# cgmb/euler

Measured on AMD Instinct MI355X. Metric: cells*steps/sec of sim_step() (frames incl. the PCG pressure projection) + pressure-solve HBM GB/s vs roofline, higher is better.
Workload: dtype f64

## Files before the change

euler_amd/__init__.py:

```python
import ctypes as C
import os

import numpy as np

_HERE = os.path.dirname(os.path.abspath(__file__))
LIB_PATH = os.path.join(_HERE, "lib", "libeuler_hip.so")

DOT_AUTO, DOT_SEQUENTIAL, DOT_TREE = 0, 1, 2
PRECOND_IC0, PRECOND_JACOBI, PRECOND_IC0_TILE, PRECOND_IC0_TILE2, PRECOND_IC0_TILE_MG = 0, 1, 2, 3, 4
(OPT_P_STEPS, OPT_TILE_STORE_AS, OPT_TILE_REVERSE, OPT_RESIDENT_CAP, OPT_GRID4_MIN_CELLS, OPT_SLAB_FUSION, OPT_RCCL_SMALL, OPT_RCCL_NO_EXCHANGE, OPT_MARKERS_ROWMAJOR,
 OPT_SA_RUN, OPT_NO_INTERIOR, OPT_BUILD_GATHER, OPT_RESIDENT_FORCE_TIMEOUT, OPT_MG_SPLIT_LEVEL, OPT_MG_SPLIT_ACTIVE, OPT_MARKERS_TWO_PASS, OPT_BUILD_TWO_PASS,
 OPT_VELOCITY_TWO_PASS, OPT_NO_TILE_MAP, OPT_PROFILE_STRIDE, OPT_TILE_STORE_Z, OPT_ADVECT_RK2, OPT_ADVECT_MACCORMACK) = range(1, 24)
SWEEP_AUTO, SWEEP_BAND, SWEEP_SIMPLE = 0, 1, 2
PCG_F64, PCG_F32 = 0, 1
RESIDENT_AUTO, RESIDENT_OFF = 0, 1
IMAGE_COVERAGE, IMAGE_DYE, IMAGE_SPEED = 0, 1, 2
EDIT_SOLID, EDIT_CLEAR, EDIT_SINK, EDIT_SOURCE, EDIT_FILL, EDIT_DRAIN = range(6)
OVERVIEW_DTYPE = np.dtype({"names": ["cells", "solid", "sink", "water", "marks", "max_speed2", "dye"],
                           "formats": [np.uint32, np.uint32, np.uint32, np.uint32, np.uint32, np.float32, (np.uint64, 3)],
                           "offsets": [0, 4, 8, 12, 16, 20, 24], "itemsize": 48})
DIAG_CROWDED = 8
DIAG_DTYPE = np.dtype({"names": ["cells", "fluid", "markers", "crowded", "mass_x", "mass_y", "div_l1", "ke_hi", "ke_lo", "count_max", "nonfinite", "max_div", "max_speed2"],
                       "formats": [np.uint64] * 9 + [np.uint32, np.uint32, np.float32, np.float32],
                       "offsets": [0, 8, 16, 24, 32, 40, 48, 56, 64, 72, 76, 80, 84], "itemsize": 88})
FLOW_PRESSURE = 1
PAINT_VORTICITY, PAINT_PRESSURE, PAINT_SPEED = 0, 1, 2
FLOW_DTYPE = np.dtype({"names": ["cells", "water", "nodes", "nonfinite", "u_pos", "u_neg", "v_pos", "v_neg", "w_pos", "w_neg", "p_sum", "max_speed2", "max_abs_w", "max_p", "reserved"],
# ... 891 lines not shown
```

euler_amd/csrc/driver.hip:

```cpp
#include "euler_dev.h"
#include "k_mg.h"

#include <math.h>
#include <stdarg.h>
#include <stdlib.h>
#include <string.h>

#include <vector>

int eu_launch_build_system(euler_sim* S, float dt);
int eu_launch_velocity_update(euler_sim* S, float dt, int finish);
int eu_pressure_current(euler_sim* S);
int eu_unskew(euler_sim* S, const void* skew, void* rowmajor, int elem_bytes);
int eu_unskew_fluid(euler_sim* S, const double* skew, double* rowmajor);
double* eu_current_search_direction(euler_sim* S);
int eu_launch_tile_table(euler_sim* S);
int eu_skew(euler_sim* S, const void* rowmajor, void* skew, int elem_bytes);
int eu_set_source_count(euler_sim* S, size_t nsrc);

static thread_local char g_err[512] = "";

void eu_set_error(const char* fmt, ...) {
  va_list ap;
  va_start(ap, fmt);
// ... 108 lines not shown

bool eu_resident_eligible(const euler_sim* S) {
  if (S->res_disabled || S->cfg.resident == EULER_RESIDENT_OFF) return false;
  if (S->cfg.precond != EULER_PRECOND_IC0_TILE || S->tile_w != 16 || S->cfg.sweep_mode == EULER_SWEEP_SIMPLE || S->cfg.dot_mode != EULER_DOT_TREE) return false;
  if (S->has_comm || S->slab_on || S->p2p_on) return false;
  const int cap = eu_resident_capacity(const_cast<euler_sim*>(S), S->cfg.pcg_precision == EULER_PCG_F32);
  if (S->cfg.pcg_precision == EULER_PCG_F32) return cap > 0 && S->geom.nbands * (S->geom.T / 16) <= 4 * cap;
  return cap > 0;
}
extern "C" int euler_resident_info(euler_sim* S, uint64_t out[3]) {
  if (!S || !out) return EULER_EINVAL;
  out[0] = eu_resident_eligible(S) ? 1 : 0; out[1] = S->res_solves; out[2] = S->res_fallbacks;
  return EULER_OK;
}

extern "C" int euler_set_option(euler_sim* S, int32_t key, int64_t value) {
  if (!S || key <= 0 || key >= EULER_OPT__COUNT) { eu_set_error("euler_set_option: unknown key %d", (int)key); return EULER_EINVAL; }
  bool ok = true;
  const char* when = nullptr;
  switch (key) {
    case EULER_OPT_P_STEPS: ok = value == 2 || value == 4 || value == 8; break;
    case EULER_OPT_SA_RUN: ok = value == 8 || value == 16 || value == 32;
      if (ok && value != 8 && (S->has_comm || eu_is_two_level(S))) when = "on a handle without a communicator, in the parity or the plain tile-local mode (the others run runs of 8)";
      break;
    case EULER_OPT_RCCL_SMALL: ok = value >= 0 && value <= 2; if (S->rccl) when = "before euler_set_comm_rccl"; break;
    case EULER_OPT_RCCL_NO_EXCHANGE: ok = value == 0 || value == 1; if (S->rccl) when = "before euler_set_comm_rccl"; break;
    case EULER_OPT_SLAB_FUSION: ok = value == 0 || value == 1; if (S->p2p_on) when = "before euler_p2p_connect"; break;
    case EULER_OPT_RESIDENT_CAP: case EULER_OPT_GRID4_MIN_CELLS: case EULER_OPT_RESIDENT_FORCE_TIMEOUT: ok = value >= 0; break;
    case EULER_OPT_MG_SPLIT_LEVEL: ok = value >= -1 && value < 12; break;
    case EULER_OPT_PROFILE_STRIDE: ok = value >= 1 && value <= 1024; break;
    case EULER_OPT_MG_SPLIT_ACTIVE: ok = false; break;
    case EULER_OPT_ADVECT_RK2: ok = value == 0 || value == 1;
// ... 15 lines not shown
      eu_set_error("euler_set_option: EULER_OPT_ADVECT_MACCORMACK needs %zu bytes of scratch", 2 * bytes);
      return EULER_ENOMEM;
    }
    S->mc_u = a; S->mc_v = b;
  }
  if (key == EULER_OPT_P_STEPS || key == EULER_OPT_SA_RUN) {
    int rcp = eu_pressure_current(S);
    if (rcp) return rcp;
  }
  S->opt[key] = value;
  if (key == EULER_OPT_P_STEPS || key == EULER_OPT_SA_RUN) S->s_ring_n = 0;
  if (key == EULER_OPT_MG_SPLIT_LEVEL) { eu_mg_split_release(S); S->opt[EULER_OPT_MG_SPLIT_ACTIVE] = 0; }
  return EULER_OK;
}
extern "C" int euler_get_option(euler_sim* S, int32_t key, int64_t* value) {
  if (!S || !value || key <= 0 || key >= EULER_OPT__COUNT) { eu_set_error("euler_get_option: unknown key %d", (int)key); return EULER_EINVAL; }
  *value = S->opt[key];
  return EULER_OK;
}

static const char* eu_precond_combination(const euler_sim* S, int precond, int tile_w, int has_comm, int slab_on, int p2p_on) {
  const bool coarse = precond == EULER_PRECOND_IC0_TILE2 || precond == EULER_PRECOND_IC0_TILE_MG;
  if (!coarse) return nullptr;
  if (tile_w != 16 || S->cfg.sweep_mode == EULER_SWEEP_SIMPLE) return "the coarse-correction preconditioners run on tiles of 16 records with the band schedule";
  if (precond == EULER_PRECOND_IC0_TILE2 && (has_comm || slab_on)) return "EULER_PRECOND_IC0_TILE2 runs on one GPU (row slabs: EULER_PRECOND_IC0_TILE_MG)";
  if (precond == EULER_PRECOND_IC0_TILE_MG && has_comm && (!slab_on || p2p_on)) return "EULER_PRECOND_IC0_TILE_MG with several ranks: row-slab handles without mailboxes only";
  return nullptr;
}

extern "C" int euler_set_precond(euler_sim* S, int32_t precond, int32_t tile_records) {
  if (!S || precond < EULER_PRECOND_IC0 || precond > EULER_PRECOND_IC0_TILE_MG) { eu_set_error("euler_set_precond: bad argument"); return EULER_EINVAL; }
// ... 884 lines not shown
```

euler_amd/csrc/k_grid.hip:

```cpp
#include "k_pcg.h"
#include "k_transport.h"

#include <stdlib.h>

__device__ __forceinline__ void dt_from_maxima(MarkerState* ms, float frame_time_left, unsigned int mu_bits, unsigned int mv_bits) {
  const float mu = __uint_as_float(mu_bits), mv = __uint_as_float(mv_bits);
  const float max_distance = 0.75f * EU_H;
  const float max_velocity = sqrtf(mu + mv);
  ms->dt = fminf(max_distance / max_velocity, frame_time_left);
  ms->max_u2_bits = 0u;
  ms->max_v2_bits = 0u;
}
template <bool FUSE_DT>
__global__ __launch_bounds__(256) void k_maxsq(const float* __restrict__ u, const float* __restrict__ v,
                                               int X, int Y, MarkerState* ms, int y0, int y1, float frame_time_left) {
  float mu = 0.f, mv = 0.f;
  const bool vec = (X & 3) == 0;
  for (int yq = y0 + 4 * (int)blockIdx.x; yq < y1; yq += 4 * (int)gridDim.x) {
    if (vec) {
      for (int x = 4 * (int)threadIdx.x; x < X; x += 4 * 256) {
        float4 a[4], b[4];
#pragma unroll
        for (int r = 0; r < 4; ++r) {
          const int y = yq + r < y1 ? yq + r : y1 - 1;
// ... 662 lines not shown
    const bool f1 = count[i + X] != 0;
    float o = 0.f;
    if (solid[i] | solid[i + X]) o = 0.f;
    else if (f0 | f1) {
      double p1 = p[skew_index(g, x, y + 1)];
      if (f1 && p1 < 0.0) p1 = 0.0;
      o = vin[i] + (neg_inv * (float)(p1 - p0)) * dt;
    }
    vout[i] = o;
  }
}

struct VuRing { const double* s[8]; int n, steps, use; };
#define VU_W 48
#define VU_ILP 4
__global__ __launch_bounds__(256) void k_velocity_update_para(const float* __restrict__ uin, const float* __restrict__ vin, float* __restrict__ uout, float* __restrict__ vout,
                                                              const double* __restrict__ p, const uint8_t* __restrict__ mask, const uint8_t* __restrict__ count,
                                                              const uint8_t* __restrict__ solid, SkewGeom g, float dt, const PcgScalars* sc, VuRing ring, MarkerState* ms,
                                                              int band_lo, int do_max, int skip_zero,
                                                              const uint8_t* __restrict__ tmap, int tnx) {
  __shared__ double sp[65][VU_W + 1];
  __shared__ float s_mu[4], s_mv[4];
  const int units = g.T / VU_W;
  const size_t blk = eu_xcd_block();
  const int band = band_lo + (int)(blk / units), t0 = (int)(blk % units) * VU_W;
  const int X = g.X, Y = g.Y, tid = threadIdx.x;
  if (skip_zero && tmap && eu_tiles_idle_cur(tmap, tnx, band, t0 > 63 ? (t0 - 63) >> 6 : 0, (t0 + VU_W - 1) >> 6, true)) return;
  int cnt = 0, from = 0;
  if (ring.use && sc->nonzero && sc->iters > 0) {
    const int n_it = sc->iters;
    from = n_it - 1 >= ring.steps ? (n_it - 1) / ring.steps * ring.steps : 0;
    cnt = n_it - from;
  }
  double al[8];
  const double* sq[8];
#pragma unroll
  for (int j = 0; j < 8; ++j) { const int it = from + (j < cnt ? j : 0); al[j] = sc->alpha_hist[it & 7]; sq[j] = ring.s[it % ring.n]; }
  const size_t ebase = ((size_t)band * g.TS + (size_t)t0) * 64;
  static_assert((64 * VU_W) % (256 * VU_ILP) == 0, "whole rounds of VU_ILP elements per thread");
  for (int c0 = tid; c0 < 64 * VU_W; c0 += 256 * VU_ILP) {
    uint8_t m[VU_ILP];
    double pv[VU_ILP];
    bool any = false;
#pragma unroll
    for (int u = 0; u < VU_ILP; ++u) { m[u] = mask[ebase + (size_t)(c0 + 256 * u)]; any = any || (m[u] & CM_FLUID); }
    if (__any(any)) {
#pragma unroll
      for (int u = 0; u < VU_ILP; ++u) pv[u] = p[ebase + (size_t)(c0 + 256 * u)];
#pragma unroll
      for (int j = 0; j < 8; ++j)
        if (j < cnt) {
          double sv[VU_ILP];
#pragma unroll
          for (int u = 0; u < VU_ILP; ++u) sv[u] = sq[j][ebase + (size_t)(c0 + 256 * u)];
// ... 156 lines not shown
  if (!mode) return EULER_OK;
  eu_vd_pressure_made_current(&S->vd);
  if (mode == 1) { int rc = eu_launch_finish_p(S); if (rc) return rc; }
  LAUNCH(S, KC_VELOCITY_UPDATE, k_clamp_p, dim3(eu_blocks(S->e_cnt, 256 * 4, 4096)), dim3(256), S->p, S->cellmask, S->e_lo, S->e_cnt);
  return EULER_OK;
}
int eu_launch_velocity_update(euler_sim* S, float dt, int finish) {
  const bool one_pass = (!S->has_comm || S->slab_on) && S->opt[EULER_OPT_VELOCITY_TWO_PASS] == 0 && (!S->slab_on || !finish);
  if (one_pass) {
    VuRing ring;
    for (int k = 0; k < 8; ++k) ring.s[k] = S->s_ring[k < S->s_ring_n ? k : 0];
    ring.n = S->s_ring_n > 0 ? S->s_ring_n : 1; ring.steps = ring.n; ring.use = finish && S->s_ring_n > 0;
    if (!ring.use) for (int k = 0; k < 8; ++k) ring.s[k] = S->p;
    const int do_max = S->slab_on ? 0 : 1;
    if (eu_vd_update_clears_maxima(&S->vd, do_max)) HIPCHK(hipMemsetAsync(&S->ms->max_u2_bits, 0, 2 * sizeof(unsigned int), S->stream));
    LAUNCH(S, KC_VELOCITY_UPDATE, k_velocity_update_para, dim3((unsigned)((size_t)(S->band_hi - S->band_lo) * (S->geom.T / VU_W))), dim3(256), S->utmp, S->vtmp, S->u, S->v, S->p, S->cellmask,
           S->count, S->solid, S->geom, dt, S->sc, ring, S->ms, S->band_lo, do_max, eu_vd_update_skips_zeros(&S->vd, S->slab_on),
           eu_tile_map_on(S) ? (const uint8_t*)S->tmap : (const uint8_t*)nullptr, S->tmap_nx);
    eu_vd_velocity_updated(&S->vd, 1, ring.use, do_max);
    return EULER_OK;
  }
  if (finish) { int rc = eu_launch_finish_p(S); if (rc) return rc; }
  dim3 grid((S->X + 63) / 64, (S->row_hi - S->row_lo + 3) / 4);
  LAUNCH(S, KC_VELOCITY_UPDATE, k_velocity_update, grid, dim3(256), S->utmp, S->vtmp, S->u, S->v, S->p, S->count,
         S->solid, S->geom, dt, S->row_lo, S->row_hi);
  eu_vd_velocity_updated(&S->vd, 0, 0, 0);
  return EULER_OK;
}

template <typename T>
__global__ __launch_bounds__(256) void k_unskew(const T* __restrict__ skew, T* __restrict__ rowmajor, SkewGeom g, int y0, int y1) {
// ... 33 lines not shown
```

euler_amd/csrc/k_pcg.h:

```cpp
#pragma once

#include "euler_dev.h"
#include "k_mg.h"

#define COMM_CALL(expr) do { if ((expr) != 0) { eu_set_error("communicator callback failed: %s", #expr); return EULER_ECOMM; } } while (0)
#define LOC(ptr) ((ptr) + S->e_lo)
enum { SW_FACTOR = 0, SW_FORWARD = 1, SW_BACKWARD = 2 };

int eu_launch_build_system(euler_sim* S, float dt);
int eu_launch_velocity_update(euler_sim* S, float dt, int finish);
int eu_launch_band_ranges(euler_sim* S);
int eu_launch_sweep(euler_sim* S, int op, int cls, int force, int fin_qq = -1);
int eu_launch_factor_tile(euler_sim* S, int force);
int eu_launch_precond_tile(euler_sim* S, int rupd, int sweeps, int fin_dot, int force, double alpha, bool r_only = false, int zform = -1);
int eu_launch_search_apply(euler_sim* S, int it);
int eu_launch_finish_p(euler_sim* S);
int eu_launch_dot(euler_sim* S, const double* a, const double* b, int fin_op, int force);
int eu_comm_exchange(euler_sim* S, double* send_lo, double* send_hi, double* recv_lo, double* recv_hi, int count, double* small, int nsmall);
int eu_comm_finish(euler_sim* S, int fin_op, int is_max, int force);
int eu_comm_halo_two(euler_sim* S, double* a, double* b);
bool tile_recompute(const euler_sim* S);
int p_steps(const euler_sim* S);

enum { FIN_SIGMA_INIT = 0, FIN_ALPHA, FIN_RNORM, FIN_BETA, FIN_STORE_ONLY, FIN_TO_COMM };
#define FIN_VIA_P2P 0x100

static inline bool tile_fused(const euler_sim* S) { return eu_is_tile(S) && S->cfg.sweep_mode != EULER_SWEEP_SIMPLE; }
static inline bool ghost_mode(const euler_sim* S) { return S->has_comm && !S->p2p_on && tile_fused(S); }
enum { XR_ZSEND_LO = 0, XR_ZSEND_HI, XR_ZRECV_LO, XR_ZRECV_HI, XR_GS_LO0, XR_GS_LO1, XR_GS_HI0, XR_GS_HI1 };
// ... 189 lines not shown
  const unsigned int* list;
  const double* table;
  PcgScalars* sc;
  int force;
  double alpha_arg;
  double* pair_slot;
  double *zsend_lo, *zsend_hi;
  int edge_lo, edge_hi;
  int reverse;
  double* cpart;
  int cshift;
  int cmode, cnx, cny;
  const double *gs_lo, *gs_hi;
  int zform;
  double *zhalo, *zrows;
};

__device__ __forceinline__ double factor_step(double aa, double own, double nbv) {
  const double cl = -1.0 * own, cb = -1.0 * nbv;
  double e = aa - cl * cl - cb * cb;
  if (e < 0.25 * aa) e = (aa != 0.0) ? aa : 1.0;
  return 1.0 / sqrt(e);
}

template <int CTRL>
__device__ __forceinline__ double dpp_move(double v) {
  const int lo = __builtin_amdgcn_update_dpp(0, __double2loint(v), CTRL, 0xf, 0xf, true);
  const int hi = __builtin_amdgcn_update_dpp(0, __double2hiint(v), CTRL, 0xf, 0xf, true);
  return __hiloint2double(hi, lo);
}
// ... 8 lines not shown
```

euler_amd/csrc/k_pcg.hip:

```cpp
#include "k_pcg.h"

#include <cmath>
#include <vector>

template <bool IS_MAX>
__global__ __launch_bounds__(RED_THREADS) void k_reduce_final(const double* __restrict__ partial, int n, PcgScalars* sc,
                                                              int op, int force) {
  if (!force && pcg_idle(sc)) return;
  double v = 0.0;
  for (int i = threadIdx.x; i < n; i += RED_THREADS) {
    const double w = partial[i];
    if (IS_MAX) v = w > v ? w : v; else v += w;
  }
  v = IS_MAX ? block_max(v) : block_sum(v);
  if (threadIdx.x == 0) pcg_scalar_step(sc, op, v);
}

template <bool EDGES>
__global__ __launch_bounds__(RED_THREADS) void k_dot_partial(const double* __restrict__ a, const double* __restrict__ b,
                                                             const uint8_t* __restrict__ mask, size_t S,
                                                             double* __restrict__ partial, PcgScalars* sc, int force,
                                                             unsigned int* counter, int fin_op, int TS, int nb_local, int edges) {
  if (!force && pcg_idle(sc)) return;
  const size_t chunk = (((S + gridDim.x - 1) / gridDim.x) + 1) & ~(size_t)1;
// ... 49 lines not shown
      for (int grp = 0; grp < SEQ_TILE / 64; ++grp) {
        if (any[buf][grp] == 0ull) continue;
        const double* pp = &prod[buf][grp * 64];
        double v[64];
#pragma unroll
        for (int k = 0; k < 64; ++k) v[k] = pp[k];
#pragma unroll
        for (int k = 0; k < 64; ++k) total += v[k];
      }
    }
    __syncthreads();
  }
  if (threadIdx.x == 0) pcg_scalar_step(sc, op, total);
}

__global__ __launch_bounds__(RED_THREADS) void k_apply_a(const double* __restrict__ s, double* __restrict__ z,
                                                         const uint8_t* __restrict__ mask, SkewGeom g,
                                                         double* __restrict__ partial, PcgScalars* sc, int force,
                                                         unsigned int* counter, int fin_op) {
  if (!force && pcg_idle(sc)) return;
  const size_t S = g.S;
  const size_t chunk = (((S + gridDim.x - 1) / gridDim.x) + 127) & ~(size_t)127;
  const size_t lo = (size_t)blockIdx.x * chunk, hi = lo + chunk < S ? lo + chunk : S;
  double t = 0.0;
  for (size_t i = lo + 2 * (size_t)threadIdx.x; i < hi; i += 2 * RED_THREADS) {
    const unsigned int mm = *reinterpret_cast<const unsigned short*>(mask + i);
    const unsigned int m0 = mm & 0xff, m1 = mm >> 8;
    if (!((m0 | m1) & CM_FLUID)) continue;
    const sw_d2 c = *reinterpret_cast<const sw_d2*>(s + i);
    const int l = (int)((i & 127) >> 1);
// ... 28 lines not shown
        v = v - s[up];
      } else {
        v = v - 0.0;
      }
      v = v - ((m1 & CM_LEFT) ? c.x : 0.0);
      if (m1 & CM_DOWN) {
        size_t dn = i - 2;
        if (l == 0) { int band, tt, ll; skew_decode(g, i + 1, band, tt, ll); dn = skew_index(g, tt, 64 * band - 1); }
        v = v - s[dn];
      } else {
        v = v - 0.0;
      }
      o.y = v;
      t += v * c.y;
    }
    if ((m0 & m1) & CM_FLUID) *reinterpret_cast<sw_d2*>(z + i) = o;
    else if (m0 & CM_FLUID) z[i] = o.x;
    else z[i + 1] = o.y;
  }
  t = block_sum(t);
  if (fin_op >= 0) block_finish<false>(t, partial, counter, sc, fin_op);
}

__global__ __launch_bounds__(RED_THREADS) void k_update_pr(double* __restrict__ p, double* __restrict__ r,
                                                           const double* __restrict__ s, const double* __restrict__ z,
                                                           const uint8_t* __restrict__ mask, size_t S,
                                                           double* __restrict__ partial, PcgScalars* sc, int force,
                                                           double alpha_arg, unsigned int* counter, int fin_op) {
  if (!force && pcg_idle(sc)) return;
  const double alpha = force ? alpha_arg : sc->alpha;
// ... 224 lines not shown

static inline bool dot_rides_in_sweep(const euler_sim* S) { return S->cfg.precond == EULER_PRECOND_IC0 && S->cfg.sweep_mode != EULER_SWEEP_SIMPLE && !S->has_comm && S->cfg.dot_mode != EULER_DOT_SEQUENTIAL; }
static int launch_precondition(euler_sim* S, int force, int fin_dot = -1) {
  if (S->cfg.precond == EULER_PRECOND_JACOBI) {
    LAUNCH(S, KC_JACOBI, k_jacobi, dim3(eu_blocks(S->e_cnt, 256 * 4, 4096)), dim3(256), LOC(S->r), LOC(S->z), LOC(S->cellmask),
           S->e_cnt, S->sc, force);
    return fin_dot >= 0 ? eu_launch_dot(S, S->z, S->r, fin_dot, force) : EULER_OK;
  }
  const bool ride = fin_dot >= 0 && dot_rides_in_sweep(S);
  int rc = eu_launch_sweep(S, SW_FORWARD, KC_FORWARD_SOLVE, force, ride ? fin_dot : -1);
  if (rc) return rc;
  if ((rc = eu_launch_sweep(S, SW_BACKWARD, KC_BACKWARD_SOLVE, force))) return rc;
  return fin_dot >= 0 && !ride ? eu_launch_dot(S, S->z, S->r, fin_dot, force) : EULER_OK;
}

static int launch_apply_a_and_alpha(euler_sim* S, int force) {
  const bool seq = S->cfg.dot_mode == EULER_DOT_SEQUENTIAL && !S->has_comm;
  if (S->has_comm && ghost_mode(S) && !force) {
    const int X = S->X, nbk = (X + 255) / 256;
    const bool coarse = eu_is_two_level(S);
    if (S->band_lo > 0) {
      HIPCHK(hipMemcpyAsync(xrow(S, XR_GS_LO0), xrow(S, XR_ZRECV_LO), (size_t)X * 8, hipMemcpyDeviceToDevice, S->stream));
      if (coarse) { int rc = eu_launch_coarse_add_row(S, xrow(S, XR_GS_LO0), 64 * S->band_lo - 1); if (rc) return rc; }
      hipLaunchKernelGGL(k_unpack_row, dim3(nbk), dim3(256), 0, S->stream, S->s, xrow(S, XR_GS_LO0), S->geom, S->band_lo - 1, 63);
    }
    if (S->band_hi < S->geom.nbands) {
      HIPCHK(hipMemcpyAsync(xrow(S, XR_GS_HI0), xrow(S, XR_ZRECV_HI), (size_t)X * 8, hipMemcpyDeviceToDevice, S->stream));
      if (coarse) { int rc = eu_launch_coarse_add_row(S, xrow(S, XR_GS_HI0), 64 * S->band_hi); if (rc) return rc; }
      hipLaunchKernelGGL(k_unpack_row, dim3(nbk), dim3(256), 0, S->stream, S->s, xrow(S, XR_GS_HI0), S->geom, S->band_hi, 0);
    }
    S->gs_cur = 0;
  } else if (S->has_comm) { int rc = comm_halo_s(S); if (rc) return rc; }
  SkewGeom gl = S->geom;
  gl.S = S->e_cnt;
  double* out = tile_fused(S) ? S->q : S->z;
  LAUNCH(S, KC_APPLY_A, k_apply_a, dim3(loc_red_blocks(S)), dim3(RED_THREADS), LOC(S->s), LOC(out), LOC(S->cellmask), gl,
         S->partial, S->sc, force, S->red_counter, seq ? -1 : fin_or_comm(S, FIN_ALPHA));
  if (seq)
    LAUNCH(S, KC_DOT, k_dot_sequential, dim3(1), dim3(256), out, S->s, S->cellmask, S->geom, S->sc, (int)FIN_ALPHA, force);
  return S->has_comm ? eu_comm_finish(S, FIN_ALPHA, 0, force) : EULER_OK;
}

int p_steps(const euler_sim* S) {
  if (S->p2p_on || sa_run(S) != 8) return 2;
  return (int)S->opt[EULER_OPT_P_STEPS];
}
static int ring_begin(euler_sim* S) {
  const int n = p_steps(S);
  if (!S->s_base[0]) { S->s_base[0] = S->s; S->s_base[1] = S->s2; }
  if (n > 2) { S->s = S->s_base[0]; S->s2 = S->s_base[1]; }
  else if (S->s != S->s_base[0] && S->s != S->s_base[1]) { S->s = S->s_base[0]; S->s2 = S->s_base[1]; }
// ... 93 lines not shown
    }
  }
  return EULER_OK;
}

static int project_first_direction(euler_sim* S, Solve& v) {
  int rc;
  const bool tile = tile_fused(S), two_level = tile && eu_is_two_level(S);
  if (two_level && S->has_comm && !(eu_is_mg(S) && ghost_mode(S) && S->slab_on)) {
    eu_set_error("coarse-correction preconditioners with several ranks: EULER_PRECOND_IC0_TILE_MG on row slabs without mailboxes only");
    return EULER_EINVAL;
  }
  if (two_level && (rc = eu_launch_coarse_setup(S))) return rc;
  if (two_level && (rc = eu_launch_coarse_consistent(S))) return rc;
  v.zr = tile && tile_z_begin(S);
  if (tile) {
    if ((rc = eu_launch_factor_tile(S, 0))) return rc;
    if ((rc = eu_launch_precond_tile(S, 0, 1, FIN_SIGMA_INIT, 0, 0.0))) return rc;
  } else {
  if (S->cfg.precond != EULER_PRECOND_JACOBI && (rc = eu_launch_sweep(S, SW_FACTOR, KC_PRECON_FACTOR, 0))) return rc;
  if ((rc = launch_precondition(S, 0, FIN_SIGMA_INIT))) return rc;
  }
  if ((rc = ring_begin(S))) return rc;
  if (first_direction_folded(S)) {
    const PcgScalars& ps = v.prev;
    if (ps.nonzero && !(std::isfinite(ps.alpha) && std::isfinite(ps.beta) && std::isfinite(ps.rnorm) && std::isfinite(ps.sigma) && std::isfinite(ps.zs)))
      for (int k = 0; k < S->s_ring_n; ++k) HIPCHK(hipMemsetAsync(S->s_ring[k] + S->skew_off, 0, S->Sw * sizeof(double), S->stream));
  }
  else if (two_level) { if ((rc = eu_launch_coarse_search_init(S))) return rc; }
  else
  LAUNCH(S, KC_UPDATE_SEARCH, k_update_search<true>, dim3(eu_blocks(S->e_cnt, 256 * 4, 4096)), dim3(256), LOC(S->s), LOC(S->z),
         LOC(S->cellmask), S->e_cnt, S->sc, 0, 0.0);
  if (S->has_comm && eu_p2p_has_neighbour_arrays(S)) {
    const int y0 = S->band_lo > 0 ? 64 * S->band_lo : -1, y1 = S->band_hi < S->geom.nbands ? 64 * S->band_hi - 1 : -1;
    LAUNCH(S, KC_UPDATE_SEARCH, k_publish_edge_rows, dim3((S->X + 255) / 256, 2), dim3(256), S->s, S->geom, y0, y1, S->sc);
  }
  if (S->s_ring_n == 2) HIPCHK(hipMemsetAsync(LOC(S->s2), 0, S->e_cnt * sizeof(double), S->stream));
  S->s_stale = 1;
  return EULER_OK;
}

static int project_iterate(euler_sim* S, Solve& v) {
  int rc;
  HIPCHK(hipMemcpyAsync(S->sc_host, S->sc, sizeof(PcgScalars), hipMemcpyDeviceToHost, S->stream));
  HIPCHK(hipStreamSynchronize(S->stream));
  const int poll = S->cfg.pcg_poll_interval > 0 ? S->cfg.pcg_poll_interval : 8;
  const int max_it = S->cfg.max_iterations;
  const bool tile = tile_fused(S), fold0 = first_direction_folded(S);
  int it = 0, chunk = 0;
  bool stop = !S->sc_host->nonzero;
  S->s_none = stop ? 1 : 0;
  while (it < max_it && !stop) {
    int chunk_end = it + poll;
    if (!v.drain_poll && v.pred_iters > 0 && it < v.pred_iters + poll && chunk_end > v.pred_iters - 2) {
      const int lo = v.pred_iters - 2 < chunk_end ? v.pred_iters - 2 : chunk_end;
      chunk_end = lo > it + 2 ? lo : it + 2;
    }
    if (chunk_end > max_it) chunk_end = max_it;
    for (; it < chunk_end; ++it) {
      S->prof_iter = it;
      const bool fused = it > 0 || fold0;
      if (it == 0 && fold0) { S->s = S->s_ring[S->s_ring_n - 1]; S->s2 = S->s_ring[0]; }
      if ((rc = fused ? eu_launch_search_apply(S, it) : launch_apply_a_and_alpha(S, 0))) return rc;
      if (tile) {
        S->prof_iter = it;
        const int nx = it + 1, steps = S->s_ring_n;
        const bool next_odd = !(nx >= steps && nx % steps == 0);
        const int zform = v.zr && it + 1 < max_it ? (it + 2 < max_it && next_odd ? 1 : 0) : -1;
        if ((rc = eu_launch_precond_tile(S, 1, it + 1 < max_it, FIN_BETA, 0, 0.0, false, zform))) return rc;
        S->z_halo_last = zform == 1;
        v.zr_ran = v.zr_ran || zform == 1;
        continue;
      }
      S->tile_as_override = fused ? S->q : S->z;
      rc = eu_launch_precond_tile(S, 1, 0, -1, 0, 0.0, true);
      S->tile_as_override = nullptr;
      if (rc) return rc;
      if (it + 1 < max_it) {
// ... 67 lines not shown
  if (eu_is_two_level(S) && (op == EULER_OP_PRECON_FACTOR || op == EULER_OP_FORWARD_SOLVE || op == EULER_OP_BACKWARD_SOLVE)) {
    eu_set_error("euler_pcg_op: the preconditioner of EULER_PRECOND_IC0_TILE2 / _MG is not available as a single operation (select EULER_PRECOND_IC0_TILE for its tile level)");
    return EULER_EINVAL;
  }
  switch (op) {
    case EULER_OP_BUILD_SYSTEM:
      LAUNCH(S, KC_MISC, k_pcg_reset, dim3(1), dim3(1), S->sc, S->cfg.tol, S->cfg.max_iterations);
      eu_launch_build_system(S, dt);
      break;
    case EULER_OP_PRECON_FACTOR: if (tile_fused(S)) eu_launch_factor_tile(S, 1); else eu_launch_sweep(S, SW_FACTOR, KC_PRECON_FACTOR, 1); break;
    case EULER_OP_FORWARD_SOLVE: if (!tile_fused(S)) eu_launch_sweep(S, SW_FORWARD, KC_FORWARD_SOLVE, 1); break;
    case EULER_OP_BACKWARD_SOLVE:
      if (tile_fused(S)) eu_launch_precond_tile(S, 0, 1, FIN_STORE_ONLY, 1, 0.0); else eu_launch_sweep(S, SW_BACKWARD, KC_BACKWARD_SOLVE, 1);
      break;
    case EULER_OP_APPLY_A:
      LAUNCH(S, KC_APPLY_A, k_apply_a, dim3(S->red_blocks), dim3(RED_THREADS), S->s, S->z, S->cellmask, S->geom,
             S->partial, S->sc, 1, S->red_counter, -1);
      break;
    case EULER_OP_DOT_ZR: eu_launch_dot(S, S->z, S->r, FIN_STORE_ONLY, 1); break;
    case EULER_OP_DOT_ZS: eu_launch_dot(S, S->z, S->s, FIN_STORE_ONLY, 1); break;
    case EULER_OP_INF_NORM_R:
      LAUNCH(S, KC_UPDATE_PR, k_inf_norm, dim3(S->red_blocks), dim3(RED_THREADS), S->r, S->cellmask, SS, S->partial);
      LAUNCH(S, KC_REDUCE_FINAL, k_reduce_final<true>, dim3(1), dim3(RED_THREADS), S->partial, S->red_blocks, S->sc,
             (int)FIN_STORE_ONLY, 1);
      break;
    case EULER_OP_UPDATE_PR:
      LAUNCH(S, KC_UPDATE_PR, k_update_pr, dim3(S->red_blocks), dim3(RED_THREADS), S->p, S->r, S->s, S->z, S->cellmask,
             SS, S->partial, S->sc, 1, a, S->red_counter, -1);
      break;
    case EULER_OP_UPDATE_SEARCH:
      LAUNCH(S, KC_UPDATE_SEARCH, k_update_search<false>, dim3(eu_blocks(SS, 256 * 4, 4096)), dim3(256), S->s, S->z,
// ... 10 lines not shown
```

euler_amd/csrc/k_tile.hip:

```cpp
#include "k_pcg.h"

#include <type_traits>

#define PT_THREADS 256
__device__ __forceinline__ void tile_block_reduce(double& mx, double& sm) {
  __shared__ double s_mx[PT_THREADS / 64], s_sm[PT_THREADS / 64];
  mx = eu_wave_max(mx);
  sm = eu_wave_sum(sm);
  __syncthreads();
  if ((threadIdx.x & 63) == 0) { s_mx[threadIdx.x >> 6] = mx; s_sm[threadIdx.x >> 6] = sm; }
  __syncthreads();
  if (threadIdx.x == 0) {
    mx = s_mx[0]; sm = s_sm[0];
    for (int k = 1; k < PT_THREADS / 64; ++k) { mx = s_mx[k] > mx ? s_mx[k] : mx; sm += s_sm[k]; }
  }
}

__global__ __launch_bounds__(64) void k_tile_table(double* __restrict__ tab) {
  const int lane = threadIdx.x & 63;
  double own = 0.0, out = 0.0;
  sw_d2 pp[8];
#pragma unroll
  for (int j = 0; j < 16; ++j) {
    const double nbv = wave_shift_inject<DPP_WAVE_SHR1>(out, 0.0);
// ... 230 lines not shown
      if (W == 16 && a.zform == 1) {
        double* h = a.zhalo + ((size_t)band * ntb + k) * 128;
        h[lane] = qq[0].x;
        h[64 + lane] = qq[W / 2 - 1].y;
        if (lane == 0 || lane == 63) {
          double* row = a.zrows + ((size_t)band * 2 + (lane == 63 ? 1 : 0)) * a.g.X;
#pragma unroll
          for (int j = 0; j < W; ++j) {
            const int x = k * W + j - lane;
            if (x >= 0 && x < a.g.X) row[x] = (j & 1) ? qq[j >> 1].y : qq[j >> 1].x;
          }
        }
      } else {
#pragma unroll
        for (int P = 0; P < W / 2; ++P) *reinterpret_cast<sw_d2*>(a.z + base + P * 128) = qq[P];
      }
      if (band == a.edge_lo || band == a.edge_hi) {
        const bool lo = band == a.edge_lo && lane == 0, hi = band == a.edge_hi && lane == 63;
#pragma unroll
        for (int j = 0; j < W; ++j) {
          const double zv = (j & 1) ? qq[j >> 1].y : qq[j >> 1].x;
          const int x_lo = k * W + j, x_hi = k * W + j - 63;
          if (lo && x_lo < a.g.X) a.zsend_lo[x_lo] = zv;
          if (hi && x_hi >= 0 && x_hi < a.g.X) a.zsend_hi[x_hi] = zv;
        }
      }
    };
    if (W == 16 && interior) run(yes_t()); else run(no_t());
  }
  tile_block_reduce(mx, dsum);
// ... 38 lines not shown
}
static TileArgs make_tile_args(euler_sim* S, int force) {
  TileArgs a;
  a.g = S->geom; a.mask = S->cellmask; a.pre = S->precon; a.r = S->r; a.as = S->tile_as_override ? S->tile_as_override : S->q; a.z = S->z;
  a.band_lo = S->band_lo; a.nb_local = S->band_hi - S->band_lo;
  a.rupd = 0; a.sweeps = 1; a.fin_dot = -1;
  a.via = S->has_comm ? (S->p2p_on ? (int)FIN_VIA_P2P : (int)FIN_TO_COMM) : 0;
  a.part_max = S->partial; a.part_dot = S->partial2; a.counter = S->red_counter; a.sc = S->sc; a.force = force; a.alpha_arg = 0.0;
  a.pair_slot = S->pair_buf + 2 * (S->has_comm ? S->comm.rank : 0);
  a.list = !force ? S->chunk_list : nullptr;
  a.table = S->tile_table;
  a.zsend_lo = a.zsend_hi = nullptr; a.edge_lo = a.edge_hi = -1;
  a.reverse = S->opt[EULER_OPT_TILE_REVERSE] != 0;
  a.cpart = nullptr; a.cshift = 0; a.cmode = 0; a.cnx = a.cny = 0;
  a.gs_lo = a.gs_hi = nullptr;
  a.zform = -1; a.zhalo = S->zhalo; a.zrows = S->zrows;
  if (ghost_mode(S)) {
    if (S->band_lo > 0) { a.zsend_lo = xrow(S, XR_ZSEND_LO); a.edge_lo = S->band_lo; }
    if (S->band_hi < S->geom.nbands) { a.zsend_hi = xrow(S, XR_ZSEND_HI); a.edge_hi = S->band_hi - 1; }
  }
  return a;
}
static inline unsigned tile_blocks(const euler_sim* S, int w) {
  return eu_blocks((size_t)(S->band_hi - S->band_lo) * (S->geom.T / w), PT_THREADS / 64, 2048);
}
typedef void (*TileKernel)(TileArgs);
int eu_launch_factor_tile(euler_sim* S, int force) {
  const TileKernel k = S->tile_w == 8 ? k_factor_tile<8> : S->tile_w == 32 ? k_factor_tile<32> : k_factor_tile<16>;
  LAUNCH(S, KC_PRECON_FACTOR, k, dim3(tile_blocks(S, S->tile_w)), dim3(PT_THREADS), make_tile_args(S, force));
  return EULER_OK;
}
int eu_launch_precond_tile(euler_sim* S, int rupd, int sweeps, int fin_dot, int force, double alpha, bool r_only, int zform) {
  const bool seq = S->cfg.dot_mode == EULER_DOT_SEQUENTIAL && !S->has_comm;
  TileArgs a = make_tile_args(S, force);
  a.rupd = rupd; a.sweeps = sweeps; a.fin_dot = (seq || !sweeps) ? -1 : fin_dot; a.alpha_arg = alpha;
  a.zform = zform;
  const bool two_level = eu_is_two_level(S) && sweeps && !r_only && !force && a.list != nullptr;
  const int fin_real = a.fin_dot;
  if (two_level) {
    const bool mg = eu_is_mg(S);
    a.cpart = mg ? S->mg_part : S->cc_part; a.cshift = mg ? 0 : S->coarse_shift;
    a.cmode = mg ? 2 : 1; a.cnx = mg ? S->mg_nx[0] : 0; a.cny = mg ? S->mg_ny[0] : 0;
    if (a.fin_dot >= 0) a.fin_dot = FIN_STORE_ONLY;
  }
  double* xsmall = S->pair_buf;
  int nsmall = 2;
  bool split = false;
  if (two_level && a.via == FIN_TO_COMM) {
    split = eu_is_mg(S) && ghost_mode(S) && eu_mg_split(S);
    nsmall = eu_coarse_comm_slots(S);
    if (nsmall < 0) return EULER_ENOMEM;
// ... 42 lines not shown
```

include/euler.h:

```cpp
#ifndef EULER_H
#define EULER_H

#include <stddef.h>
#include <stdint.h>

#ifdef __cplusplus
extern "C" {
#endif

#define EULER_ABI_VERSION 2

enum {
  EULER_OK = 0,
  EULER_EINVAL = -1,
  EULER_ENOMEM = -2,
  EULER_EIO = -3,
  EULER_EHIP = -4,
  EULER_ESTATE = -5,
  EULER_ETIMEOUT = -6,
  EULER_ECOMM = -7
};

enum {
  EULER_DOT_AUTO = 0,
// ... 367 lines not shown
  EULER_OPT_MARKERS_ROWMAJOR = 9,
  EULER_OPT_SA_RUN = 10,
  EULER_OPT_NO_INTERIOR = 11,
  EULER_OPT_BUILD_GATHER = 12,
  EULER_OPT_RESIDENT_FORCE_TIMEOUT = 13,
  EULER_OPT_MG_SPLIT_LEVEL = 14,
  EULER_OPT_MG_SPLIT_ACTIVE = 15,
  EULER_OPT_MARKERS_TWO_PASS = 16,
  EULER_OPT_BUILD_TWO_PASS = 17,
  EULER_OPT_VELOCITY_TWO_PASS = 18,
  EULER_OPT_NO_TILE_MAP = 19,
  EULER_OPT_PROFILE_STRIDE = 20,
  EULER_OPT_TILE_STORE_Z = 21,
  EULER_OPT_ADVECT_RK2 = 22,
  EULER_OPT_ADVECT_MACCORMACK = 23,
  EULER_OPT__COUNT
};
int euler_set_option(euler_sim* sim, int32_t key, int64_t value);
int euler_get_option(euler_sim* sim, int32_t key, int64_t* value);

int euler_comm_calls(euler_sim* sim, uint64_t out[5]);

#define EULER_P2P_HANDLE_BYTES 256
int euler_p2p_export(euler_sim* sim, void* handle_out, int32_t cap);
int euler_p2p_connect(euler_sim* sim, const void* handles, int32_t nranks);
int euler_p2p_disconnect(euler_sim* sim);
int euler_p2p_calls(euler_sim* sim, uint64_t out[2]);
int euler_set_stream(euler_sim* sim, void* hip_stream);
int euler_slab_info(euler_sim* sim, int32_t* band_lo, int32_t* band_hi, int32_t* nbands);

// ... 16 lines not shown
```

Baseline: 190.9 million.

## Fuse first search-direction copy into precond pass, skip dead apply-A store, pair velocity loads

The first preconditioner tile pass now also writes z into the initial search direction, which removes the separate k_update_search copy kernel. When the tile recompute path will not read the apply-A output, the first apply-A launch drops its store. The velocity update kernel now loads mask and pressure in pairs (16-bit mask, double2 pressure) with a warp-wide skip when no fluid is present. All three are on by default and each has an option to restore the old path. The costs are an extra store stream inside the precond kernel and some correctness coupling between when the ring is set up and the tile flags.

```diff
diff --git a/euler_amd/__init__.py b/euler_amd/__init__.py
--- a/euler_amd/__init__.py
+++ b/euler_amd/__init__.py
@@ -11,6 +11,7 @@
 (OPT_P_STEPS, OPT_TILE_STORE_AS, OPT_TILE_REVERSE, OPT_RESIDENT_CAP, OPT_GRID4_MIN_CELLS, OPT_SLAB_FUSION, OPT_RCCL_SMALL, OPT_RCCL_NO_EXCHANGE, OPT_MARKERS_ROWMAJOR,
  OPT_SA_RUN, OPT_NO_INTERIOR, OPT_BUILD_GATHER, OPT_RESIDENT_FORCE_TIMEOUT, OPT_MG_SPLIT_LEVEL, OPT_MG_SPLIT_ACTIVE, OPT_MARKERS_TWO_PASS, OPT_BUILD_TWO_PASS,
  OPT_VELOCITY_TWO_PASS, OPT_NO_TILE_MAP, OPT_PROFILE_STRIDE, OPT_TILE_STORE_Z, OPT_ADVECT_RK2, OPT_ADVECT_MACCORMACK) = range(1, 24)
+OPT_S0_COPY, OPT_APPLY_A_STORE, OPT_VELOCITY_SCALAR_LOADS = 25, 26, 27
 SWEEP_AUTO, SWEEP_BAND, SWEEP_SIMPLE = 0, 1, 2
 PCG_F64, PCG_F32 = 0, 1
 RESIDENT_AUTO, RESIDENT_OFF = 0, 1
diff --git a/euler_amd/csrc/driver.hip b/euler_amd/csrc/driver.hip
--- a/euler_amd/csrc/driver.hip
+++ b/euler_amd/csrc/driver.hip
@@ -146,8 +146,9 @@
   return EULER_OK;
 }
 
+static inline bool eu_option_key(int32_t key) { return key > 0 && key < EULER_OPT__COUNT && key != 24; }
 extern "C" int euler_set_option(euler_sim* S, int32_t key, int64_t value) {
-  if (!S || key <= 0 || key >= EULER_OPT__COUNT) { eu_set_error("euler_set_option: unknown key %d", (int)key); return EULER_EINVAL; }
+  if (!S || !eu_option_key(key)) { eu_set_error("euler_set_option: unknown key %d", (int)key); return EULER_EINVAL; }
   bool ok = true;
   const char* when = nullptr;
   switch (key) {
@@ -193,7 +194,7 @@
   return EULER_OK;
 }
 extern "C" int euler_get_option(euler_sim* S, int32_t key, int64_t* value) {
-  if (!S || !value || key <= 0 || key >= EULER_OPT__COUNT) { eu_set_error("euler_get_option: unknown key %d", (int)key); return EULER_EINVAL; }
+  if (!S || !value || !eu_option_key(key)) { eu_set_error("euler_get_option: unknown key %d", (int)key); return EULER_EINVAL; }
   *value = S->opt[key];
   return EULER_OK;
 }
diff --git a/euler_amd/csrc/k_grid.hip b/euler_amd/csrc/k_grid.hip
--- a/euler_amd/csrc/k_grid.hip
+++ b/euler_amd/csrc/k_grid.hip
@@ -700,6 +700,8 @@
 struct VuRing { const double* s[8]; int n, steps, use; };
 #define VU_W 48
 #define VU_ILP 4
+#define VU_PAIR_ILP 3
+template <bool PAIRS>
 __global__ __launch_bounds__(256) void k_velocity_update_para(const float* __restrict__ uin, const float* __restrict__ vin, float* __restrict__ uout, float* __restrict__ vout,
                                                               const double* __restrict__ p, const uint8_t* __restrict__ mask, const uint8_t* __restrict__ count,
                                                               const uint8_t* __restrict__ solid, SkewGeom g, float dt, const PcgScalars* sc, VuRing ring, MarkerState* ms,
@@ -724,6 +726,42 @@
   for (int j = 0; j < 8; ++j) { const int it = from + (j < cnt ? j : 0); al[j] = sc->alpha_hist[it & 7]; sq[j] = ring.s[it % ring.n]; }
   const size_t ebase = ((size_t)band * g.TS + (size_t)t0) * 64;
   static_assert((64 * VU_W) % (256 * VU_ILP) == 0, "whole rounds of VU_ILP elements per thread");
+  static_assert((32 * VU_W) % (256 * VU_PAIR_ILP) == 0, "whole rounds of VU_PAIR_ILP pairs per thread");
+  if (PAIRS) {
+    for (int c0 = 2 * tid; c0 < 64 * VU_W; c0 += 512 * VU_PAIR_ILP) {
+      unsigned int mm[VU_PAIR_ILP];
+      sw_d2 pv[VU_PAIR_ILP];
+      bool any = false;
+#pragma unroll
+      for (int u = 0; u < VU_PAIR_ILP; ++u) {
+        mm[u] = *reinterpret_cast<const unsigned short*>(mask + ebase + (size_t)(c0 + 512 * u));
+        any = any || ((mm[u] | (mm[u] >> 8)) & CM_FLUID);
+      }
+      if (__any(any)) {
+#pragma unroll
+        for (int u = 0; u < VU_PAIR_ILP; ++u) pv[u] = *reinterpret_cast<const sw_d2*>(p + ebase + (size_t)(c0 + 512 * u));
+#pragma unroll
+        for (int j = 0; j < 8; ++j)
+          if (j < cnt) {
+            sw_d2 sv[VU_PAIR_ILP];
+#pragma unroll
+            for (int u = 0; u < VU_PAIR_ILP; ++u) sv[u] = *reinterpret_cast<const sw_d2*>(sq[j] + ebase + (size_t)(c0 + 512 * u));
+#pragma unroll
+            for (int u = 0; u < VU_PAIR_ILP; ++u) { pv[u].x = pv[u].x + sv[u].x * al[j]; pv[u].y = pv[u].y + sv[u].y * al[j]; }
+          }
+      } else {
+#pragma unroll
+        for (int u = 0; u < VU_PAIR_ILP; ++u) pv[u] = sw_d2{0.0, 0.0};
+      }
+#pragma unroll
+      for (int u = 0; u < VU_PAIR_ILP; ++u) {
+        const int c = c0 + 512 * u;
+        double* row = &sp[(c & 127) >> 1][2 * (c >> 7)];
+        row[0] = (mm[u] & CM_FLUID) ? (pv[u].x < 0.0 ? 0.0 : pv[u].x) : 0.0;
+        row[1] = ((mm[u] >> 8) & CM_FLUID) ? (pv[u].y < 0.0 ? 0.0 : pv[u].y) : 0.0;
+      }
+    }
+  } else
   for (int c0 = tid; c0 < 64 * VU_W; c0 += 256 * VU_ILP) {
     uint8_t m[VU_ILP];
     double pv[VU_ILP];
@@ -910,7 +948,7 @@
     if (!ring.use) for (int k = 0; k < 8; ++k) ring.s[k] = S->p;
     const int do_max = S->slab_on ? 0 : 1;
     if (eu_vd_update_clears_maxima(&S->vd, do_max)) HIPCHK(hipMemsetAsync(&S->ms->max_u2_bits, 0, 2 * sizeof(unsigned int), S->stream));
-    LAUNCH(S, KC_VELOCITY_UPDATE, k_velocity_update_para, dim3((unsigned)((size_t)(S->band_hi - S->band_lo) * (S->geom.T / VU_W))), dim3(256), S->utmp, S->vtmp, S->u, S->v, S->p, S->cellmask,
+    LAUNCH(S, KC_VELOCITY_UPDATE, S->opt[EULER_OPT_VELOCITY_SCALAR_LOADS] ? k_velocity_update_para<false> : k_velocity_update_para<true>, dim3((unsigned)((size_t)(S->band_hi - S->band_lo) * (S->geom.T / VU_W))), dim3(256), S->utmp, S->vtmp, S->u, S->v, S->p, S->cellmask,
            S->count, S->solid, S->geom, dt, S->sc, ring, S->ms, S->band_lo, do_max, eu_vd_update_skips_zeros(&S->vd, S->slab_on),
            eu_tile_map_on(S) ? (const uint8_t*)S->tmap : (const uint8_t*)nullptr, S->tmap_nx);
     eu_vd_velocity_updated(&S->vd, 1, ring.use, do_max);
diff --git a/euler_amd/csrc/k_pcg.h b/euler_amd/csrc/k_pcg.h
--- a/euler_amd/csrc/k_pcg.h
+++ b/euler_amd/csrc/k_pcg.h
@@ -12,7 +12,7 @@
 int eu_launch_band_ranges(euler_sim* S);
 int eu_launch_sweep(euler_sim* S, int op, int cls, int force, int fin_qq = -1);
 int eu_launch_factor_tile(euler_sim* S, int force);
-int eu_launch_precond_tile(euler_sim* S, int rupd, int sweeps, int fin_dot, int force, double alpha, bool r_only = false, int zform = -1);
+int eu_launch_precond_tile(euler_sim* S, int rupd, int sweeps, int fin_dot, int force, double alpha, bool r_only = false, int zform = -1, double* s0 = nullptr);
 int eu_launch_search_apply(euler_sim* S, int it);
 int eu_launch_finish_p(euler_sim* S);
 int eu_launch_dot(euler_sim* S, const double* a, const double* b, int fin_op, int force);
@@ -232,6 +232,7 @@
   const double *gs_lo, *gs_hi;
   int zform;
   double *zhalo, *zrows;
+  double* s0;
 };
 
 __device__ __forceinline__ double factor_step(double aa, double own, double nbv) {
diff --git a/euler_amd/csrc/k_pcg.hip b/euler_amd/csrc/k_pcg.hip
--- a/euler_amd/csrc/k_pcg.hip
+++ b/euler_amd/csrc/k_pcg.hip
@@ -87,6 +87,7 @@
   if (threadIdx.x == 0) pcg_scalar_step(sc, op, total);
 }
 
+template <bool STORE>
 __global__ __launch_bounds__(RED_THREADS) void k_apply_a(const double* __restrict__ s, double* __restrict__ z,
                                                          const uint8_t* __restrict__ mask, SkewGeom g,
                                                          double* __restrict__ partial, PcgScalars* sc, int force,
@@ -145,6 +146,7 @@
       o.y = v;
       t += v * c.y;
     }
+    if (!STORE) continue;
     if ((m0 & m1) & CM_FLUID) *reinterpret_cast<sw_d2*>(z + i) = o;
     else if (m0 & CM_FLUID) z[i] = o.x;
     else z[i + 1] = o.y;
@@ -399,7 +401,7 @@
   return fin_dot >= 0 && !ride ? eu_launch_dot(S, S->z, S->r, fin_dot, force) : EULER_OK;
 }
 
-static int launch_apply_a_and_alpha(euler_sim* S, int force) {
+static int launch_apply_a_and_alpha(euler_sim* S, int force, bool store = true) {
   const bool seq = S->cfg.dot_mode == EULER_DOT_SEQUENTIAL && !S->has_comm;
   if (S->has_comm && ghost_mode(S) && !force) {
     const int X = S->X, nbk = (X + 255) / 256;
@@ -419,7 +421,7 @@
   SkewGeom gl = S->geom;
   gl.S = S->e_cnt;
   double* out = tile_fused(S) ? S->q : S->z;
-  LAUNCH(S, KC_APPLY_A, k_apply_a, dim3(loc_red_blocks(S)), dim3(RED_THREADS), LOC(S->s), LOC(out), LOC(S->cellmask), gl,
+  LAUNCH(S, KC_APPLY_A, store || seq ? k_apply_a<true> : k_apply_a<false>, dim3(loc_red_blocks(S)), dim3(RED_THREADS), LOC(S->s), LOC(out), LOC(S->cellmask), gl,
          S->partial, S->sc, force, S->red_counter, seq ? -1 : fin_or_comm(S, FIN_ALPHA));
   if (seq)
     LAUNCH(S, KC_DOT, k_dot_sequential, dim3(1), dim3(256), out, S->s, S->cellmask, S->geom, S->sc, (int)FIN_ALPHA, force);
@@ -543,21 +545,23 @@
   if (two_level && (rc = eu_launch_coarse_setup(S))) return rc;
   if (two_level && (rc = eu_launch_coarse_consistent(S))) return rc;
   v.zr = tile && tile_z_begin(S);
+  const bool s0_in_pass = v.zr && S->opt[EULER_OPT_S0_COPY] == 0;
+  if (s0_in_pass && (rc = ring_begin(S))) return rc;
   if (tile) {
     if ((rc = eu_launch_factor_tile(S, 0))) return rc;
-    if ((rc = eu_launch_precond_tile(S, 0, 1, FIN_SIGMA_INIT, 0, 0.0))) return rc;
+    if ((rc = eu_launch_precond_tile(S, 0, 1, FIN_SIGMA_INIT, 0, 0.0, false, -1, s0_in_pass ? S->s : nullptr))) return rc;
   } else {
   if (S->cfg.precond != EULER_PRECOND_JACOBI && (rc = eu_launch_sweep(S, SW_FACTOR, KC_PRECON_FACTOR, 0))) return rc;
   if ((rc = launch_precondition(S, 0, FIN_SIGMA_INIT))) return rc;
   }
-  if ((rc = ring_begin(S))) return rc;
+  if (!s0_in_pass && (rc = ring_begin(S))) return rc;
   if (first_direction_folded(S)) {
     const PcgScalars& ps = v.prev;
     if (ps.nonzero && !(std::isfinite(ps.alpha) && std::isfinite(ps.beta) && std::isfinite(ps.rnorm) && std::isfinite(ps.sigma) && std::isfinite(ps.zs)))
       for (int k = 0; k < S->s_ring_n; ++k) HIPCHK(hipMemsetAsync(S->s_ring[k] + S->skew_off, 0, S->Sw * sizeof(double), S->stream));
   }
   else if (two_level) { if ((rc = eu_launch_coarse_search_init(S))) return rc; }
-  else
+  else if (!s0_in_pass)
   LAUNCH(S, KC_UPDATE_SEARCH, k_update_search<true>, dim3(eu_blocks(S->e_cnt, 256 * 4, 4096)), dim3(256), LOC(S->s), LOC(S->z),
          LOC(S->cellmask), S->e_cnt, S->sc, 0, 0.0);
   if (S->has_comm && eu_p2p_has_neighbour_arrays(S)) {
@@ -576,6 +580,7 @@
   const int poll = S->cfg.pcg_poll_interval > 0 ? S->cfg.pcg_poll_interval : 8;
   const int max_it = S->cfg.max_iterations;
   const bool tile = tile_fused(S), fold0 = first_direction_folded(S);
+  const bool as0_store = !(v.zr && tile && tile_recompute(S) && S->opt[EULER_OPT_APPLY_A_STORE] == 0 && max_it > 1);
   int it = 0, chunk = 0;
   bool stop = !S->sc_host->nonzero;
   S->s_none = stop ? 1 : 0;
@@ -590,7 +595,7 @@
       S->prof_iter = it;
       const bool fused = it > 0 || fold0;
       if (it == 0 && fold0) { S->s = S->s_ring[S->s_ring_n - 1]; S->s2 = S->s_ring[0]; }
-      if ((rc = fused ? eu_launch_search_apply(S, it) : launch_apply_a_and_alpha(S, 0))) return rc;
+      if ((rc = fused ? eu_launch_search_apply(S, it) : launch_apply_a_and_alpha(S, 0, as0_store))) return rc;
       if (tile) {
         S->prof_iter = it;
         const int nx = it + 1, steps = S->s_ring_n;
@@ -688,7 +693,7 @@
       if (tile_fused(S)) eu_launch_precond_tile(S, 0, 1, FIN_STORE_ONLY, 1, 0.0); else eu_launch_sweep(S, SW_BACKWARD, KC_BACKWARD_SOLVE, 1);
       break;
     case EULER_OP_APPLY_A:
-      LAUNCH(S, KC_APPLY_A, k_apply_a, dim3(S->red_blocks), dim3(RED_THREADS), S->s, S->z, S->cellmask, S->geom,
+      LAUNCH(S, KC_APPLY_A, k_apply_a<true>, dim3(S->red_blocks), dim3(RED_THREADS), S->s, S->z, S->cellmask, S->geom,
              S->partial, S->sc, 1, S->red_counter, -1);
       break;
     case EULER_OP_DOT_ZR: eu_launch_dot(S, S->z, S->r, FIN_STORE_ONLY, 1); break;
diff --git a/euler_amd/csrc/k_tile.hip b/euler_amd/csrc/k_tile.hip
--- a/euler_amd/csrc/k_tile.hip
+++ b/euler_amd/csrc/k_tile.hip
@@ -268,6 +268,10 @@
       } else {
 #pragma unroll
         for (int P = 0; P < W / 2; ++P) *reinterpret_cast<sw_d2*>(a.z + base + P * 128) = qq[P];
+        if (W == 16 && !RECOMP && CMODE == 0 && a.s0) {
+#pragma unroll
+          for (int P = 0; P < W / 2; ++P) *reinterpret_cast<sw_d2*>(a.s0 + base + P * 128) = qq[P];
+        }
       }
       if (band == a.edge_lo || band == a.edge_hi) {
         const bool lo = band == a.edge_lo && lane == 0, hi = band == a.edge_hi && lane == 63;
@@ -336,7 +340,7 @@
   a.reverse = S->opt[EULER_OPT_TILE_REVERSE] != 0;
   a.cpart = nullptr; a.cshift = 0; a.cmode = 0; a.cnx = a.cny = 0;
   a.gs_lo = a.gs_hi = nullptr;
-  a.zform = -1; a.zhalo = S->zhalo; a.zrows = S->zrows;
+  a.zform = -1; a.zhalo = S->zhalo; a.zrows = S->zrows; a.s0 = nullptr;
   if (ghost_mode(S)) {
     if (S->band_lo > 0) { a.zsend_lo = xrow(S, XR_ZSEND_LO); a.edge_lo = S->band_lo; }
     if (S->band_hi < S->geom.nbands) { a.zsend_hi = xrow(S, XR_ZSEND_HI); a.edge_hi = S->band_hi - 1; }
@@ -352,11 +356,11 @@
   LAUNCH(S, KC_PRECON_FACTOR, k, dim3(tile_blocks(S, S->tile_w)), dim3(PT_THREADS), make_tile_args(S, force));
   return EULER_OK;
 }
-int eu_launch_precond_tile(euler_sim* S, int rupd, int sweeps, int fin_dot, int force, double alpha, bool r_only, int zform) {
+int eu_launch_precond_tile(euler_sim* S, int rupd, int sweeps, int fin_dot, int force, double alpha, bool r_only, int zform, double* s0) {
   const bool seq = S->cfg.dot_mode == EULER_DOT_SEQUENTIAL && !S->has_comm;
   TileArgs a = make_tile_args(S, force);
   a.rupd = rupd; a.sweeps = sweeps; a.fin_dot = (seq || !sweeps) ? -1 : fin_dot; a.alpha_arg = alpha;
-  a.zform = zform;
+  a.zform = zform; a.s0 = s0;
   const bool two_level = eu_is_two_level(S) && sweeps && !r_only && !force && a.list != nullptr;
   const int fin_real = a.fin_dot;
   if (two_level) {
diff --git a/include/euler.h b/include/euler.h
--- a/include/euler.h
+++ b/include/euler.h
@@ -405,6 +405,9 @@
   EULER_OPT_TILE_STORE_Z = 21,
   EULER_OPT_ADVECT_RK2 = 22,
   EULER_OPT_ADVECT_MACCORMACK = 23,
+  EULER_OPT_S0_COPY = 25,
+  EULER_OPT_APPLY_A_STORE = 26,
+  EULER_OPT_VELOCITY_SCALAR_LOADS = 27,
   EULER_OPT__COUNT
 };
 int euler_set_option(euler_sim* sim, int32_t key, int64_t value);
```

New measurement: 193.8 million, median of 6. About the same (+1.5%).
